# violetdenim/c3dgs

Measured on AMD Instinct MI355X. Metric: raster views/sec fwd+bwd @1920x1080, higher is better.
Workload: dtype f32; 1 GPU; BASELINE.json configs[2]: synth-v1 3M Gaussians, SH deg 3, indexed-camera rasterizer (QAT inner loop), mark_visible+fwd+bwd, 1 view/step/GPU; gaussians=3000000, width=1920, height=1080, sh_codebook=304096, gaussian_codebook=754096, parallelism=replicas x1

## Files before the change

__graft_entry__.py:

```python
import os
import subprocess
import sys

ROOT = os.path.dirname(os.path.abspath(__file__))
if ROOT not in sys.path:
    sys.path.insert(0, ROOT)


def build() -> None:
    from c3dgs_amd import build as hip_build
    lib = hip_build.build()
    assert os.path.exists(lib)
    for variant in hip_build.VARIANTS:
        assert os.path.exists(hip_build.build_variant(variant))
    subprocess.check_call(["make", "-C", os.path.join(ROOT, "oracle"), "-s"])
    import c3dgs_amd
    from c3dgs_amd import _lib
    L = _lib.lib()
    assert L.c3dgs_abi_version() == 4


def smoke() -> None:
    import numpy as np
    import torch
    from tests import cases, gpu_util, synth
    from oracle import oracle as orc

    assert torch.cuda.is_available(), "smoke() needs a GPU"
    torch.cuda.set_device(0)
    for name in ("base", "indexed"):
        inp, cam, indexed = cases.make_case(name)
        st = cases.oracle_forward(inp, cam)
        fw = gpu_util.hip_forward(inp, cam, indexed)
        u = gpu_util.unpack(fw)
        np.testing.assert_array_equal(u["radii"], st.radii)
        np.testing.assert_array_equal(u["keys_sorted"], st.keys_sorted)
        np.testing.assert_array_equal(u["point_list"], st.point_list)
        assert gpu_util.psnr(u["out_color"], st.out_color) >= 80.0
        dL = synth.grad_image(cam["W"], cam["H"]).numpy()
        ref = orc.rasterize_backward(st, dL)
        got = gpu_util.hip_backward(fw, dL)
        for k, v in got.items():
            if ref[k].shape == v.shape and v.size:
                err = gpu_util.rel_inf(v, ref[k])
                assert err <= 1e-4, (name, k, err)
    import c3dgs_amd
# ... 15 lines not shown
```

c3dgs_amd/build.py:

```python
import os
import subprocess
import sys
from concurrent.futures import ThreadPoolExecutor

HERE = os.path.dirname(os.path.abspath(__file__))
CSRC = os.path.join(HERE, "csrc")
OBJ = os.path.join(HERE, "build")
LIB = os.path.join(HERE, "libc3dgs_hip.so")
HIPCC = os.environ.get("HIPCC", "/opt/rocm/bin/hipcc")
ARCH = "gfx950"

COMMON = ["--offload-arch=" + ARCH, "-O3", "-fPIC", "-std=c++17", "-Wall", "-Wno-unused-function",
          "-fno-gpu-rdc", "-DNDEBUG"]
SOURCES = {
    "c_abi.hip": [],
    "c_abi_debug.hip": [],
    "preprocess.hip": ["-ffp-contract=off"],
    "backward_preprocess.hip": ["-ffp-contract=off"] + os.environ.get("C3DGS_BWDPRE_FLAGS", "").split(),
    "binning.hip": [],
    "radix_sort.hip": os.environ.get("C3DGS_SORT_FLAGS", "").split(),
    "render.hip": os.environ.get("C3DGS_RENDER_FLAGS", "-fno-slp-vectorize").split(),
    "vq.hip": ["-mllvm", "-amdgpu-mfma-vgpr-form"] + os.environ.get("C3DGS_VQ_FLAGS", "").split(),
    "draws.hip": [],
    "loss.hip": [],
    "metrics.hip": [],
    "encode.hip": [],
    "knn.hip": ["-ffp-contract=off"],
    "adam.hip": ["-ffp-contract=off"],
    "qat.hip": ["-ffp-contract=off"],
    "densify.hip": ["-ffp-contract=off"],
}
HEADERS = [os.path.join(CSRC, "common.hpp"), os.path.join(CSRC, "gsmath.hpp"), os.path.join(CSRC, "render_diag.hpp"),
           os.path.join(HERE, "..", "include", "c3dgs_hip.h"), os.path.join(HERE, "..", "include", "c3dgs_hip_debug.h")]


def _stale(target, deps):
    if not os.path.exists(target):
        return True
    t = os.path.getmtime(target)
    return any(os.path.getmtime(d) > t for d in deps)


def _compile(name, extra, verbose):
    src = os.path.join(CSRC, name)
    obj = os.path.join(OBJ, name.replace(".hip", ".o"))
    cmd = [HIPCC] + COMMON + extra + ["-c", src, "-o", obj]
    if verbose:
        print(" ".join(cmd), flush=True)
    subprocess.check_call(cmd)
    return obj


VARIANTS = {"spin1": {"radix_sort.hip": ["-DC3DGS_OS_SPIN_LIMIT=1u"]}}
def _diag(mode):
    return {src: ["-DC3DGS_DIAG", mode] for src in ("render.hip", "radix_sort.hip", "diag.hip")}


DIAG_VARIANTS = {"lanes": _diag("-DC3DGS_COUNT_LANES"), "bwdtime": _diag("-DC3DGS_BWD_TIMING"), "ostime": _diag("-DC3DGS_OS_TIMING")}


def build_variant(name, verbose=False):
    build(verbose=verbose)
    flags = {**VARIANTS, **DIAG_VARIANTS}[name]
    odir = os.path.join(HERE, "build", "variant_" + name)
    os.makedirs(odir, exist_ok=True)
    lib = os.path.join(HERE, f"libc3dgs_hip_{name}.so")
    objs, rebuilt = [], False
    for src in list(SOURCES) + [f for f in flags if f not in SOURCES]:
        extra = SOURCES.get(src, [])
        obj = os.path.join(OBJ, src.replace(".hip", ".o"))
        if src in flags:
            obj = os.path.join(odir, src.replace(".hip", ".o"))
            if _stale(obj, [os.path.join(CSRC, src)] + HEADERS + [os.path.abspath(__file__)]):
                cmd = [HIPCC] + COMMON + extra + flags[src] + ["-c", os.path.join(CSRC, src), "-o", obj]
                if verbose:
                    print(" ".join(cmd), flush=True)
                subprocess.check_call(cmd)
                rebuilt = True
        objs.append(obj)
    if rebuilt or _stale(lib, objs):
        subprocess.check_call([HIPCC, "--offload-arch=" + ARCH, "-shared", "-fPIC", "-o", lib] + objs)
    return lib


def build(force=False, verbose=False):
    os.makedirs(OBJ, exist_ok=True)
    deps_common = HEADERS + [os.path.abspath(__file__)]
    todo, objs = [], []
    for name, extra in SOURCES.items():
        obj = os.path.join(OBJ, name.replace(".hip", ".o"))
        objs.append(obj)
        if force or _stale(obj, [os.path.join(CSRC, name)] + deps_common):
            todo.append((name, extra))
    if todo:
        with ThreadPoolExecutor(max_workers=min(4, len(todo))) as ex:
            list(ex.map(lambda t: _compile(t[0], t[1], verbose), todo))
    if force or todo or _stale(LIB, objs):
        cmd = [HIPCC, "--offload-arch=" + ARCH, "-shared", "-fPIC", "-o", LIB] + objs
        if verbose:
            print(" ".join(cmd), flush=True)
        subprocess.check_call(cmd)
    return LIB


if __name__ == "__main__":
    print(build(force="--force" in sys.argv, verbose="--verbose" in sys.argv or "-v" in sys.argv))
    for flag, table in (("--variants", VARIANTS), ("--diag", DIAG_VARIANTS)):
        for v in table if flag in sys.argv else ():
            print(build_variant(v, verbose="--verbose" in sys.argv or "-v" in sys.argv))
```

c3dgs_amd/csrc/c_abi.hip:

```cpp
#include "common.hpp"
#include <cstdlib>
#include <cstring>
#include <mutex>
#include <vector>

namespace c3dgs {

static thread_local std::string g_last_error;
void set_error(const std::string& msg) { g_last_error = msg; }

enum Stage { ST_MARK_VISIBLE, ST_PREPROCESS, ST_DEPTH_SORT, ST_SCAN, ST_DUPLICATE, ST_SORT, ST_RANGES, ST_RENDER_FWD, ST_ZERO_PARTIALS,
             ST_RENDER_BWD, ST_BWD_PREPROCESS, ST_WDIST, ST_VQ_ACC, ST_VQ_APPLY, ST_LOSS_FWD, ST_LOSS_BWD,
             ST_QAT_OBSERVE, ST_QAT_CODEBOOKS, ST_QAT_VISIBLE, ST_QAT_POINTS, ST_QAT_POINTS_BWD, ST_QAT_CODEBOOKS_BWD, ST_ADAM,
             ST_KNN_SORT, ST_KNN_BOUNDS, ST_KNN_QUERY, ST_COUNT };
static const char* kStageNames[ST_COUNT] = { "mark_visible", "preprocess", "depth_sort", "scan", "duplicate_with_keys", "sort",
                                             "identify_ranges", "render_forward", "zero_partials", "render_backward",
                                             "backward_preprocess", "weighted_distance", "vq_accumulate", "vq_apply", "l1_ssim_forward",
                                             "l1_ssim_backward", "qat_observe", "qat_codebooks", "qat_visible", "qat_points",
                                             "qat_points_backward", "qat_codebooks_backward", "adam_step",
                                             "knn_sort", "knn_bounds", "knn_query" };
struct ProfRec { int stage; hipEvent_t a, b; };
static std::mutex g_prof_mu;
static bool g_prof_on = false;
static int g_prof_only = -1;
// ... 210 lines not shown
        const size_t n_sh = (grads->dL_dsh && p.sh) ? (size_t)p.SHS * p.M * 3 * sizeof(float) : 0;
        const size_t n_rot = (grads->dL_drotations && p.scales) ? (size_t)p.GS * 4 * sizeof(float) : 0;
        const size_t n_sc = (grads->dL_dscales && p.scales) ? (size_t)p.GS * 3 * sizeof(float) : 0;
        char* a_sh = (char*)grads->dL_dsh; char* a_rot = (char*)grads->dL_drotations; char* a_sc = (char*)grads->dL_dscales;
        if (n_sh && n_rot && n_sc && a_rot == a_sh + n_sh && a_sc == a_rot + n_rot) {
            const size_t n = n_sh + n_rot + n_sc;
            if (p.P > 0 && R >= 0 && ((uintptr_t)a_sh & 15u) == 0) {
                cb_zero = a_sh; cb_zero16 = n / 16;
                if (n % 16) C3DGS_HIP_TRY(hipMemsetAsync(a_sh + cb_zero16 * 16, 0, n % 16, s));
            } else {
                C3DGS_HIP_TRY(hipMemsetAsync(a_sh, 0, n, s));
            }
        } else {
            if (n_sh) C3DGS_HIP_TRY(hipMemsetAsync(a_sh, 0, n_sh, s));
            if (n_sc) C3DGS_HIP_TRY(hipMemsetAsync(a_sc, 0, n_sc, s));
            if (n_rot) C3DGS_HIP_TRY(hipMemsetAsync(a_rot, 0, n_rot, s));
        }
    }
    if (P == 0) return C3DGS_OK;
    if (!radii || !geom_buffer || !image_buffer || !dL_dout_color || (R > 0 && !binning_buffer))
        return fail(C3DGS_E_INVALID, "radii, forward buffers and dL_dout_color are required");
    if (!ws_resize) return fail(C3DGS_E_INVALID, "workspace callback is required");
    if (R < 0) return fail(C3DGS_E_INVALID, "R must be >= 0");

    const GeomPtrs g = geom_ptrs(const_cast<void*>(geom_buffer), P);
    const ImgPtrs img = img_ptrs(const_cast<void*>(image_buffer), W, H);
    const size_t ws_bytes = c3dgs_backward_workspace_bytes(P, R);
    float* partials = (float*)ws_resize(ws_user, ws_bytes);
    if (!partials) return fail(C3DGS_E_ALLOC, "backward workspace allocation failed");

    const size_t r1 = (size_t)(R > 0 ? R : 1), p256 = ((size_t)P + 1023) / 1024 * 1024;
    uint8_t* touched = (uint8_t*)partials + align_up(r1 * PARTIAL_FLOATS * sizeof(float));
    uint32_t* tile_order = img.tile_order;
    uint32_t* live_ids = (uint32_t*)(touched + align_up(r1)) + 65536;
    uint32_t* live_slots = live_ids + p256;
    uint32_t* live_count = live_slots + p256;
    { StageTimer t_(ST_ZERO_PARTIALS, s);
      launch_backward_prep(R > 0 ? W : 0, H, img, tile_order, touched, align_up(r1) / 16, R > 0 ? nullptr : cb_zero,
                           R > 0 ? 0 : cb_zero16, s); }
    if (R > 0) {
        const BinPtrs b = bin_ptrs(const_cast<void*>(binning_buffer), R, W, H);
        { StageTimer t_(ST_RENDER_BWD, s);
          launch_render_backward(W, H, img, g.splat, g.block_base, p.background, dL_dout_color, partials, touched,
                                 compact_ptrs(b, R, W, H), tile_order, cb_zero, cb_zero16, s); }
        C3DGS_STAGE("render_backward", p.debug, s);
    }
    { StageTimer t_(ST_BWD_PREPROCESS, s);
      launch_backward_preprocess(p, radii, g, partials, touched, live_count, live_ids, live_slots, *grads, s); }
    C3DGS_STAGE("backward_preprocess", p.debug, s);
    return C3DGS_OK;
}

}

using namespace c3dgs;

extern "C" {

const char* c3dgs_last_error(void) { return g_last_error.c_str(); }

int c3dgs_profile_enable(int on)
{
    std::lock_guard<std::mutex> lk(g_prof_mu);
    g_prof_on = on != 0;
    return C3DGS_OK;
}

int c3dgs_profile_only(const char* stage_name)
{
    std::lock_guard<std::mutex> lk(g_prof_mu);
    g_prof_only = -1;
    if (!stage_name || !*stage_name) return C3DGS_OK;
    for (int i = 0; i < ST_COUNT; i++)
        if (std::strcmp(stage_name, kStageNames[i]) == 0) { g_prof_only = i; return C3DGS_OK; }
    return fail(C3DGS_E_INVALID, std::string("profile_only: unknown stage ") + stage_name);
}

// ... 571 lines not shown
```

c3dgs_amd/csrc/common.hpp:

```cpp
#pragma once
#include <hip/hip_runtime.h>
#include <cstdint>
#include <cstddef>
#include <cstdio>
#include <cstring>
#include <string>

#include "../../include/c3dgs_hip.h"

namespace c3dgs {

constexpr int TILE = 16;
constexpr int TILE_PIX = 256;
constexpr int SPLAT_F4 = 3;
constexpr int PARTIAL_FLOATS = 9;

void set_error(const std::string& msg);
inline int fail(int code, const std::string& msg) { set_error(msg); return code; }

#define C3DGS_HIP_TRY(expr)                                                                         \
    do {                                                                                            \
        hipError_t e__ = (expr);                                                                    \
        if (e__ != hipSuccess)                                                                      \
            return ::c3dgs::fail(C3DGS_E_HIP, std::string(#expr) + ": " + hipGetErrorString(e__));  \
// ... 156 lines not shown
void launch_camera_from_pose(const float* pose, float inv_tan_x, float inv_tan_y, float* view, float* proj, float* campos, hipStream_t s);
void launch_mark_visible(int P, const float* means3D, const float* view, uint8_t* present, hipStream_t s);
void launch_mark_visible_pose(int P, const float* means3D, const float* pose7, uint8_t* present, hipStream_t s);
void launch_pack_codebook(const c3dgs_raster_params& p, float4* gtab, hipStream_t s);
void launch_preprocess(const c3dgs_raster_params& p, const GeomPtrs& g, int32_t* radii, uint2* ranges, const uint32_t* sort_err,
                       void* zero_span, size_t zero_n16, uint32_t* host_out, uint32_t host_seq, hipStream_t s);
void launch_depth_order_scan(int P, const GeomPtrs& g, hipStream_t s);
void launch_duplicate_with_keys(int P, const GeomPtrs& g, const BinPtrs& b, int grid_x, const uint32_t* sort_err,
                                void* zero_span, size_t zero_n16, hipStream_t s);
void launch_identify_ranges(int R, const void* keys_sorted, int key_bytes, uint2* ranges, const uint32_t* sort_err, hipStream_t s);
hipError_t run_depth_sort(void* temp, size_t temp_bytes, const uint32_t* kin, uint32_t* kout, const uint32_t* vin,
                          uint32_t* vout, int P, const uint2* rects, uint2* rects_sorted, hipStream_t s, bool ctrl_cleared = false,
                          bool rects_fit_bytes = false);
hipError_t run_tile_sort(void* temp, size_t temp_bytes, const void* kin, void* kout, int key_bytes, const uint32_t* vin,
                         uint32_t* vout, int R, int end_bit, hipStream_t s, bool ctrl_cleared = false);
size_t depth_sort_clear_bytes(int P);
size_t tile_sort_clear_bytes(int R, int end_bit, int key_bytes);
bool onesweep_enabled();
int onesweep_timed_out(hipStream_t s);
uint32_t* onesweep_error_word();
size_t onesweep_depth_temp_bytes(int P);
size_t onesweep_tile_temp_bytes(int R, int end_bit, int key_bytes = 2);
size_t onesweep_depth_clear_bytes(int P);
size_t onesweep_tile_clear_bytes(int R, int end_bit, int key_bytes);
hipError_t onesweep_depth_sort(void* temp, size_t temp_bytes, const uint32_t* kin, uint32_t* kout, const uint32_t* vin, uint32_t* vout,
                               int P, const uint2* gather_src, uint2* gather_dst, hipStream_t s, bool ctrl_cleared = false,
                               bool rects_fit_bytes = false);
hipError_t onesweep_tile_sort32(void* temp, size_t temp_bytes, const uint32_t* kin, uint32_t* kout, const uint32_t* vin, uint32_t* vout,
                                int R, int end_bit, hipStream_t s, bool ctrl_cleared = false);
hipError_t onesweep_tile_sort(void* temp, size_t temp_bytes, const uint16_t* kin, uint16_t* kout, const uint32_t* vin, uint32_t* vout,
                              int R, int end_bit, hipStream_t s, bool ctrl_cleared = false);
void launch_render_forward(int W, int H, const ImgPtrs& img, const uint32_t* point_list, const float4* splat,
                           const float* bg, float* out_color, const CompactPtrs& cl, const uint32_t* sort_err, hipStream_t s);
void launch_backward_prep(int W, int H, const ImgPtrs& img, uint32_t* tile_order, void* zero_a, size_t n16_a, void* zero_b,
                          size_t n16_b, hipStream_t s);
void launch_render_backward(int W, int H, const ImgPtrs& img, const float4* splat,
                            const uint32_t* block_base, const float* bg, const float* dL_dpix, float* partials,
                            uint8_t* touched, const CompactPtrs& cl, const uint32_t* tile_order, void* zero_span, size_t zero_n16,
                            hipStream_t s);
void launch_backward_preprocess(const c3dgs_raster_params& p, const int32_t* radii, const GeomPtrs& g,
                                float* partials, const uint8_t* touched, uint32_t* live_count, uint32_t* live_ids,
                                uint32_t* live_slots, const c3dgs_raster_grads& gr, hipStream_t s);
int launch_weighted_distance(int64_t N, int C, int K, const float* coefs, const int64_t* gather, const float* codebook,
                             float* out_dist, int64_t* out_idx, hipStream_t s, void* ws = nullptr, size_t ws_bytes = 0, int presplit = -1);
bool wd_presplit_supported(int C, int K, const float* coefs, const float* codebook, const void* ws, size_t ws_bytes);
int launch_vq_apply_split(int K, int D, float* S, float* codebook, float* entry_importance, float decay, float alpha, float eps,
                          int scale_normalize, void* ws, size_t ws_bytes, int parity, hipStream_t s);
void launch_vq_seed_words(int K, int D, void* ws, hipStream_t s);
uint32_t* vq_next_absmax_word(int K, int D, void* ws, int parity);
size_t wd_ws_bytes(int64_t N, int C, int K);
int launch_wd_debug_scores(int64_t N, int C, int K, const float* coefs, const float* codebook, float* scores, void* ws, size_t ws_bytes,
                           float* out_dist, int64_t* out_idx, hipStream_t s);
void launch_vq_accumulate(int64_t B, int K, int D, const float* x, const float* w, const int64_t* gather,
                          const int64_t* idx, const float* dist, float* S, double* dist_sum, hipStream_t s, uint32_t* clear_word = nullptr);
void launch_vq_apply(int K, int D, const float* S, float* codebook, float* entry_importance, float decay, float alpha,
                     float eps, int scale_normalize, hipStream_t s);

size_t morton_workspace_bytes(int P);
int run_morton_order(int P, const float* xyz, int64_t* codes_out, int64_t* order_out, void* workspace, hipStream_t s);
void launch_extract_rot_scale(int n, const float* cov6, float* rot, float* scale, hipStream_t s);
size_t knn_workspace_bytes(int P);
int run_knn_sort(int P, const float* xyz, void* workspace, hipStream_t s);
void launch_knn_bounds(int P, void* workspace, hipStream_t s);
void launch_knn_query(int P, const void* workspace, float* out, hipStream_t s);
void launch_adam(int n_tensors, const c3dgs_adam_tensor* tensors, double beta1, double beta2, double eps, hipStream_t s);
void launch_abs_accumulate(int64_t n, const float* g, float* acc, hipStream_t s);
void launch_densify_classify(int P, const float* accum, const float* denom, const float* scale_clone, const float* scale_split,
                             const float* scale_prune_self, const float* scale_prune_child, const float* opacity, float max_grad,
                             float dense_extent, float min_opacity, float big_extent, uint8_t* code, hipStream_t s);
size_t rows_plan_workspace_bytes(int P);
hipError_t run_rows_plan(int P, const uint8_t* code, int N, long long capacity, int32_t* src, uint8_t* kind, int32_t* draw_row,
// ... 41 lines not shown
```

c3dgs_amd/csrc/render.hip:

```cpp
#include "common.hpp"
#include "render_diag.hpp"
#include <algorithm>

namespace c3dgs {

constexpr int BATCH = 256;

__device__ __forceinline__ void prescale_conic(float4& a, float4& b)
{
    constexpr float LOG2E = 1.4426950408889634f;
    a.z *= -0.5f * LOG2E;
    a.w *= -LOG2E;
    b.x *= -0.5f * LOG2E;
}

__device__ __forceinline__ bool gaussian_alpha(float mx, float my, float ka, float kb, float kc, float op,
                                               float pxf, float pyf, float& dx, float& dy, float& G, float& alpha)
{
    dx = mx - pxf;
    dy = my - pyf;
    const float power2 = fmaf(kb, dx * dy, fmaf(kc, dy * dy, ka * (dx * dx)));
    G = __builtin_amdgcn_exp2f(power2);
    alpha = fminf(0.99f, op * G);
    return !(power2 > 0.0f) && !(alpha < 1.0f / 255.0f);
// ... 10 lines not shown
}

__device__ __forceinline__ uint32_t quadrant_mask(const float4 a, const float4 b, float tile_x0, float tile_y0)
{
    const float mx = a.x, my = a.y, ca = a.z, cb = a.w, cc = b.x, op = b.y;
    if (op < (1.0f / 255.0f) * 0.999f) return 0u;
    const float det = ca * cc - cb * cb;
    const float tau = __logf(255.0f * op) * 1.0001f + 1e-4f;
    if (!(det > 0.0f) || !(ca > 0.0f) || !(cc > 0.0f) || !(tau < 1e30f)) return 0xfu;
    const float nb_c = -cb / cc, nb_a = -cb / ca;
    uint32_t mask = 0u;
#pragma unroll
    for (int q = 0; q < 4; q++) {
        const float x0 = tile_x0 + (float)((q & 1) * 8) - 0.01f - mx, y0 = tile_y0 + (float)((q >> 1) * 8) - 0.01f - my;
        const float fmin = min_power_on_rect(ca, cb, cc, nb_c, nb_a, x0, x0 + 7.02f, y0, y0 + 7.02f);
        mask |= (uint32_t)(!(fmin > tau)) << q;
    }
    return mask;
}

__device__ __forceinline__ unsigned long long uniform_u64(unsigned long long v)
{
    const uint32_t lo = __builtin_amdgcn_readfirstlane((uint32_t)v), hi = __builtin_amdgcn_readfirstlane((uint32_t)(v >> 32));
    return ((unsigned long long)hi << 32) | lo;
}

__device__ __forceinline__ int tile_of_block(int b, int T)
{
    const int chunk = (T + 7) >> 3;
    return (b & 7) * chunk + (b >> 3);
}

__global__ void __launch_bounds__(1024) backward_prep_kernel(int T, const uint32_t* __restrict__ tile_used, uint32_t* __restrict__ order,
                                                              uint4* __restrict__ zero_a, size_t n16_a, uint4* __restrict__ zero_b, size_t n16_b)
{
    if (blockIdx.x > 0) {
        const uint4 z = make_uint4(0u, 0u, 0u, 0u);
        const size_t stride = (size_t)(gridDim.x - 1) * 1024;
        for (size_t i = (size_t)(blockIdx.x - 1) * 1024 + threadIdx.x; i < n16_a; i += stride) zero_a[i] = z;
        for (size_t i = (size_t)(blockIdx.x - 1) * 1024 + threadIdx.x; i < n16_b; i += stride) zero_b[i] = z;
        return;
    }
    if (T <= 0) return;
    auto work = [&](int i) { return tile_used[i]; };
    __shared__ uint32_t s_cnt[1024], s_w[16];
    const int t = threadIdx.x, lane = t & 63, wave = t >> 6;
    s_cnt[t] = 0;
    __syncthreads();
    for (int i = t; i < T; i += 1024) atomicAdd(&s_cnt[1023 - min(work(i) >> 3, 1023u)], 1u);
    __syncthreads();
    const uint32_t c = s_cnt[t];
    uint32_t incl = c;
#pragma unroll
    for (int o = 1; o < 64; o <<= 1) { const uint32_t v = __shfl_up(incl, o); if (lane >= o) incl += v; }
    if (lane == 63) s_w[wave] = incl;
    __syncthreads();
    uint32_t off = 0;
    for (int w = 0; w < wave; w++) off += s_w[w];
    s_cnt[t] = off + incl - c;
    __syncthreads();
    for (int i = t; i < T; i += 1024) order[atomicAdd(&s_cnt[1023 - min(work(i) >> 3, 1023u)], 1u)] = (uint32_t)i;
}

__global__ void __launch_bounds__(256)
render_forward_kernel(int W, int H, int gx, int T, const uint2* __restrict__ ranges, const uint32_t* __restrict__ point_list,
                      const float4* __restrict__ splat, const float* __restrict__ bg, float* __restrict__ out_color,
                      float* __restrict__ final_T, uint32_t* __restrict__ n_contrib, uint32_t* __restrict__ tile_used,
                      uint32_t* __restrict__ n_contrib_c, uint32_t* __restrict__ tile_used_c, uint8_t* __restrict__ cqm,
                      uint32_t* __restrict__ cid, const uint32_t* __restrict__ sort_err)
{
    const int tile = tile_of_block(blockIdx.x, T);
    if (tile >= T || (blockIdx.x >> 3) >= ((T + 7) >> 3)) return;
    __shared__ float4 s_ab[2][BATCH + 1][2];
    __shared__ float s_c[2][BATCH + 1];
    __shared__ uint32_t s_list[4][BATCH + 8];
    __shared__ int s_wdone[2][4];
// ... 181 lines not shown
__device__ __forceinline__ void reduce_columns_24(float* u, int lane)
{
    transpose_reduce_step<24, 0xB1>(u, (lane & 1) != 0);
    transpose_reduce_step<12, 0x4E>(u, (lane & 2) != 0);
}

__device__ __forceinline__ void reduce_rows_9(const float* n, float& total, float& ninth)
{
    float o[4];
    C3DGS_TR4("row_ror:8", "0x3", "0xc", o, n, n, 0, 4);
    float t8;
    asm volatile("s_nop 1\n\tv_add_f32_dpp %0, %1, %1 row_ror:8 row_mask:0xf bank_mask:0xf" : "=&v"(t8) : "v"(n[8]));
    auto s0 = __builtin_amdgcn_permlane16_swap(__float_as_uint(o[0]), __float_as_uint(o[2]), false, false);
    auto s1 = __builtin_amdgcn_permlane16_swap(__float_as_uint(o[1]), __float_as_uint(o[3]), false, false);
    auto s8 = __builtin_amdgcn_permlane16_swap(__float_as_uint(t8), __float_as_uint(t8), false, false);
    const float w0 = __uint_as_float(s0[0]) + __uint_as_float(s0[1]);
    const float w1 = __uint_as_float(s1[0]) + __uint_as_float(s1[1]);
    const float w8 = __uint_as_float(s8[0]) + __uint_as_float(s8[1]);
    auto s2 = __builtin_amdgcn_permlane32_swap(__float_as_uint(w0), __float_as_uint(w1), false, false);
    auto s9 = __builtin_amdgcn_permlane32_swap(__float_as_uint(w8), __float_as_uint(w8), false, false);
    total = __uint_as_float(s2[0]) + __uint_as_float(s2[1]);
    ninth = __uint_as_float(s9[0]) + __uint_as_float(s9[1]);
}

#ifndef C3DGS_BWD_WPE
#define C3DGS_BWD_WPE 5
#endif
__global__ void __launch_bounds__(256) __attribute__((amdgpu_waves_per_eu(C3DGS_BWD_WPE, C3DGS_BWD_WPE)))
render_backward_kernel(int W, int H, int gx, int T, const uint2* __restrict__ ranges, const uint32_t* __restrict__ tile_used_c,
                       const uint32_t* __restrict__ cid, const float4* __restrict__ splat,
                       const uint32_t* __restrict__ block_base, const float* __restrict__ bg, const float* __restrict__ final_Ts,
                       const uint32_t* __restrict__ n_contrib_c, const float* __restrict__ dL_dpixels,
                       float* __restrict__ partials, uint8_t* __restrict__ touched, const uint8_t* __restrict__ cqm,
                       const uint32_t* __restrict__ tile_order, uint4* __restrict__ zero_span, size_t zero_n16)
{
    if (zero_n16) {
        const size_t per = (zero_n16 + gridDim.x - 1) / gridDim.x, z0 = (size_t)blockIdx.x * per, z1 = min(z0 + per, zero_n16);
        for (size_t i = z0 + threadIdx.x; i < z1; i += 256) zero_span[i] = make_uint4(0u, 0u, 0u, 0u);
    }
    if ((int)blockIdx.x >= T) return;
    PhaseClock clk;
    const int tile = (int)tile_order[blockIdx.x];
    __shared__ float4 s_ab[BATCH + 1][2];
    __shared__ float s_c[BATCH + 1];
    __shared__ uint32_t s_slot[BATCH];
    __shared__ uint32_t s_list[4][BATCH / 2 + GROUP_G];
    __shared__ unsigned long long s_mask[4][4];
    __shared__ float s_part[2][BATCH][NPART];
    constexpr uint32_t REC_BYTES = 32;
    const char* rec_base = reinterpret_cast<const char*>(&s_ab[0][0]);
    const char* blue_base = reinterpret_cast<const char*>(&s_c[0]);

    const int tid = threadIdx.x, wave = tid >> 6, lane = tid & 63;
    const int tx = tile % gx, ty = tile / gx;
    const int px = tx * TILE + (wave & 1) * 8 + (lane & 7);
    const int py = ty * TILE + (wave >> 1) * 8 + (lane >> 3);
    const bool inside = px < W && py < H;
    const float pxf = (float)px, pyf = (float)py;
    const size_t pix = (size_t)W * py + px, HW = (size_t)H * W;

    const uint2 range = ranges[tile];
    const int n = (int)(range.y - range.x);
    const int used = min(n, (int)tile_used_c[tile]);
    if (used <= 0) return;
    const int rounds = (used + BATCH - 1) / BATCH;
    if (tid == 0) { s_ab[BATCH][0] = make_float4(0, 0, 0, 0); s_ab[BATCH][1] = make_float4(0, 0, 0, 0); s_c[BATCH] = 0.f; }
    for (int q = tid; q < 4 * (BATCH / 2 + GROUP_G); q += 256) (&s_list[0][0])[q] = (uint32_t)BATCH * REC_BYTES;

    const float T_final = inside ? final_Ts[pix] : 0.f;
    float Tr = T_final;
    const int last_contributor = inside ? (int)n_contrib_c[pix] : 0;
    float dpx0 = 0.f, dpx1 = 0.f, dpx2 = 0.f;
    if (inside) { dpx0 = dL_dpixels[pix]; dpx1 = dL_dpixels[HW + pix]; dpx2 = dL_dpixels[2 * HW + pix]; }
    float Sd = T_final * (bg[0] * dpx0 + bg[1] * dpx1 + bg[2] * dpx2);
    int wave_last = last_contributor;
#pragma unroll
    for (int o = 32; o > 0; o >>= 1) wave_last = max(wave_last, __shfl_xor(wave_last, o));
    wave_last = __builtin_amdgcn_readfirstlane(wave_last);
    const int beta = ((lane >> 2) & 1) * 4 + (lane & 1) * 2 + ((lane >> 1) & 1);
    const int my_m = ((lane >> 3) & 1) * 4 + ((lane >> 4) & 1) * 2 + ((lane >> 5) & 1);
    LaneCount lc;

    uint32_t next_id = 0u, next_qm = 0u;
    {
        const int p0 = used - 1 - tid;
        if (p0 >= 0) { next_id = cid[range.x + p0]; next_qm = cqm[range.x + p0]; }
    }
    clk.mark(PhaseClock::PROLOGUE);
    for (int r = 0; r < rounds; r++) {
        __syncthreads();
        clk.mark(PhaseClock::TOP_BARRIER);
        const int mypos = used - 1 - (r * BATCH + tid);
        uint32_t qm = 0u;
        if (mypos >= 0) {
            const uint32_t id = next_id;
            qm = next_qm;
            float4 a = splat[3 * (size_t)id], b = splat[3 * (size_t)id + 1];
            const float4 c = splat[3 * (size_t)id + 2];
            prescale_conic(a, b);
            const uint32_t off = __float_as_uint(c.y), lo = __float_as_uint(c.z), hi = __float_as_uint(c.w);
            const int x0 = lo & 0xffff, y0 = lo >> 16, x1 = hi & 0xffff;
            s_slot[tid] = block_base[id >> 8] + off + (uint32_t)((ty - y0) * (x1 - x0) + (tx - x0));
            s_ab[tid][0] = a; s_ab[tid][1] = b; s_c[tid] = c.x;
        }
        {
            const int npos = mypos - BATCH;
            if (npos >= 0) { next_id = cid[range.x + npos]; next_qm = cqm[range.x + npos]; }
        }
#pragma unroll
        for (int q = 0; q < 4; q++) {
            const unsigned long long bm = __ballot((qm >> q) & 1u);
            if (lane == 0) s_mask[q][wave] = bm;
        }
        clk.mark(PhaseClock::GATHER);
#pragma unroll
        for (int w = 0; w < 2; w++)
#pragma unroll
            for (int q = 0; q < NPART; q++) s_part[w][tid][q] = 0.f;
        clk.mark(PhaseClock::CLEAR);
        __syncthreads();
        clk.mark(PhaseClock::CLOSE_BARRIER);

        const int cnt = min(BATCH, used - r * BATCH);
        const int pos0 = used - 1 - r * BATCH;
        const int thr = (pos0 - last_contributor) * (int)REC_BYTES;
#pragma unroll 1
        for (int half = 0; half < 2; half++) {
        int nw = 0;
        {
            const unsigned long long lt = (1ull << lane) - 1ull;
#pragma unroll
            for (int cc = 0; cc < 2; cc++) {
                const int c = half * 2 + cc;
                unsigned long long m = uniform_u64(s_mask[wave][c]);
                const int jmin = pos0 - wave_last + 1 - c * 64;
                if (jmin >= 64) m = 0; else if (jmin > 0) m &= ~0ull << jmin;
                if ((m >> lane) & 1ull) s_list[wave][nw + (int)__popcll(m & lt)] = (uint32_t)(c * 64 + lane) * REC_BYTES;
                nw += (int)__popcll(m);
            }
            if (lane < GROUP_G) s_list[wave][nw + lane] = (uint32_t)BATCH * REC_BYTES;
            __builtin_amdgcn_fence(__ATOMIC_RELEASE, "wavefront");
            __builtin_amdgcn_wave_barrier();
            __builtin_amdgcn_fence(__ATOMIC_ACQUIRE, "wavefront");
        }
        clk.mark(PhaseClock::COMPACT);
        uint4 row0 = *reinterpret_cast<const uint4*>(&s_list[wave][0]);
        uint4 row1 = *reinterpret_cast<const uint4*>(&s_list[wave][4]);
        float4 a_n = *reinterpret_cast<const float4*>(rec_base + row0.x);
        float4 b_n = *reinterpret_cast<const float4*>(rec_base + row0.x + 16);
        float c_n = *reinterpret_cast<const float*>(blue_base + (row0.x >> 3));
        for (int k = 0; k < nw; k += GROUP_G) {
            const uint32_t* lrow = &s_list[wave][k];
            const uint32_t e[GROUP_G] = { row0.x, row0.y, row0.z, row0.w, row1.x, row1.y, row1.z, row1.w };
            float v[GROUP_G * NCOL];
// ... 23 lines not shown
                v[g * NCOL + 2] = dchannel_dcolor * dpx2;
                const float dL_dalpha = fmaf(Tr, cd, -(rinv * Sd));
                Sd = fmaf(dchannel_dcolor, cd, Sd);
                const float w = G_eff * dL_dalpha, wx = w * dx;
                v[g * NCOL + 3] = w;
                v[g * NCOL + 4] = wx;
                v[g * NCOL + 5] = wx * dx;
                if (g == 4) { C3DGS_TR4("row_half_mirror", "0x5", "0xa", u, v, v, 0, 24); }
                if (g == 5) { C3DGS_TR4("row_half_mirror", "0x5", "0xa", u, v, v, 4, 24); C3DGS_TR4("row_half_mirror", "0x5", "0xa", u, v, v, 8, 24); }
                if (g == 6) { C3DGS_TR4("row_half_mirror", "0x5", "0xa", u, v, v, 12, 24); }
                if (g == 7) { C3DGS_TR4("row_half_mirror", "0x5", "0xa", u, v, v, 16, 24); C3DGS_TR4("row_half_mirror", "0x5", "0xa", u, v, v, 20, 24); }
            }
            row0 = *reinterpret_cast<const uint4*>(lrow + GROUP_G);
            row1 = *reinterpret_cast<const uint4*>(lrow + GROUP_G + 4);
            reduce_columns_24(u, lane);
            a_n = *reinterpret_cast<const float4*>(rec_base + row0.x);
            b_n = *reinterpret_cast<const float4*>(rec_base + row0.x + 16);
            c_n = *reinterpret_cast<const float*>(blue_base + (row0.x >> 3));
            const int myj = (int)(my_off >> 5);
            const float dyb = *reinterpret_cast<const float*>(rec_base + my_off + 4) - pyf;
            float total, ninth;
            const float nine[NPART] = { u[0], u[1], u[2], u[3], u[4], u[5], dyb * u[3], dyb * u[4], (dyb * dyb) * u[3] };
            reduce_rows_9(nine, total, ninth);
            if (myj < BATCH) {
                __hip_atomic_fetch_add(&s_part[wave >> 1][myj][my_m], total, __ATOMIC_RELAXED, __HIP_MEMORY_SCOPE_WORKGROUP);
                if (lane < 8) __hip_atomic_fetch_add(&s_part[wave >> 1][myj][8], ninth, __ATOMIC_RELAXED, __HIP_MEMORY_SCOPE_WORKGROUP);
            }
        }
        lc.end_list();
        __builtin_amdgcn_fence(__ATOMIC_RELEASE, "wavefront");
        __builtin_amdgcn_wave_barrier();
        clk.mark(PhaseClock::GROUPS);
        }
        __syncthreads();
        clk.mark(PhaseClock::FLUSH_BARRIER);
        if (tid < cnt) {
            const uint32_t slot = s_slot[tid];
            float* dst = partials + (size_t)slot * NPART;
            float t[NPART];
#pragma unroll
            for (int q = 0; q < NPART; q++) t[q] = s_part[0][tid][q] + s_part[1][tid][q];
            dst[0] = t[0]; dst[1] = t[1]; dst[2] = t[2];
            dst[3] = t[3]; dst[4] = t[4]; dst[5] = t[6];
            dst[6] = t[5]; dst[7] = t[7]; dst[8] = t[8];
            touched[slot] = 1;
        }
        clk.mark(PhaseClock::FLUSH_STORES);
    }
    lc.flush(8, lane);
    clk.flush(lane);
}

void launch_backward_prep(int W, int H, const ImgPtrs& img, uint32_t* tile_order, void* zero_a, size_t n16_a, void* zero_b,
                          size_t n16_b, hipStream_t s)
{
    const int T = (W > 0 && H > 0 && tile_order) ? tiles_x(W) * tiles_y(H) : 0;
    const size_t n16 = n16_a + n16_b;
    if (T <= 0 && n16 == 0) return;
    const unsigned fill = n16 ? (unsigned)std::min<size_t>((n16 + 1023) / 1024, 1024) : 0u;
    backward_prep_kernel<<<1 + fill, 1024, 0, s>>>(T, img.tile_used_c, tile_order, (uint4*)zero_a, n16_a, (uint4*)zero_b, n16_b);
}

void launch_render_backward(int W, int H, const ImgPtrs& img, const float4* splat,
                            const uint32_t* block_base, const float* bg, const float* dL_dpix, float* partials,
                            uint8_t* touched, const CompactPtrs& cl, const uint32_t* tile_order, void* zero_span, size_t zero_n16,
                            hipStream_t s)
{
    const int gx = tiles_x(W), T = gx * tiles_y(H);
    const int grid = ((T + 7) / 8) * 8;
    render_backward_kernel<<<grid, 256, 0, s>>>(W, H, gx, T, img.ranges, img.tile_used_c, cl.cid, splat, block_base, bg, img.final_T,
                                                img.n_contrib_c, dL_dpix, partials, touched, cl.cqm, tile_order, (uint4*)zero_span,
                                                zero_span ? zero_n16 : 0);
}

}
```

c3dgs_amd/csrc/render_diag.hpp:

```cpp
#pragma once

namespace c3dgs {

#if (defined(C3DGS_COUNT_LANES) || defined(C3DGS_BWD_TIMING)) && !defined(C3DGS_DIAG)
#error "C3DGS_COUNT_LANES / C3DGS_BWD_TIMING are modes of a -DC3DGS_DIAG build"
#endif

#ifdef C3DGS_DIAG
__device__ unsigned long long g_lane_counters[16];

int read_lane_counters(unsigned long long* out16, hipStream_t s)
{
    static const unsigned long long zeros[16] = { 0 };
    if (hipStreamSynchronize(s) != hipSuccess) return 1;
    if (hipMemcpyFromSymbol(out16, HIP_SYMBOL(g_lane_counters), sizeof(zeros)) != hipSuccess) return 1;
    return hipMemcpyToSymbol(HIP_SYMBOL(g_lane_counters), zeros, sizeof(zeros)) != hipSuccess;
}
#endif

#ifdef C3DGS_COUNT_LANES
struct LaneCount {
    unsigned long long pairs = 0, slots = 0, lanes = 0, live = 0, half = 0, blk = 0, lists = 0, aux = 0;
    int nA = 0, nB = 0, nb[4] = { 0, 0, 0, 0 };
    __device__ void pair(bool real, unsigned long long used, unsigned long long aux_mask)
// ... 4 lines not shown
        lanes += __popcll(used);
        aux += __popcll(aux_mask);
        live += used != 0;
        nA += (used & 0x00000000ffffffffull) != 0;
        nB += (used & 0xffffffff00000000ull) != 0;
        nb[0] += (used & 0x000000000f0f0f0full) != 0;
        nb[1] += (used & 0x00000000f0f0f0f0ull) != 0;
        nb[2] += (used & 0x0f0f0f0f00000000ull) != 0;
        nb[3] += (used & 0xf0f0f0f000000000ull) != 0;
    }
    __device__ void end_list()
    {
        lists++;
        half += max(nA, nB);
        blk += max(max(nb[0], nb[1]), max(nb[2], nb[3]));
        nA = nB = nb[0] = nb[1] = nb[2] = nb[3] = 0;
    }
    __device__ void flush(int base, int lane)
    {
        if (lane != 0) return;
        const unsigned long long v[8] = { pairs, slots, lanes, live, half, blk, lists, aux };
        for (int q = 0; q < 8; q++) atomicAdd(&g_lane_counters[base + q], v[q]);
    }
};
#else
struct LaneCount {
    __device__ __forceinline__ void pair(bool, unsigned long long, unsigned long long) {}
    __device__ __forceinline__ void end_list() {}
    __device__ __forceinline__ void flush(int, int) {}
};
#endif

struct PhaseClock {
    enum Phase { PROLOGUE, TOP_BARRIER, GATHER, CLEAR, CLOSE_BARRIER, COMPACT, GROUPS, FLUSH_BARRIER, FLUSH_STORES, NPHASE };
#ifdef C3DGS_BWD_TIMING
    unsigned long long born = __builtin_readcyclecounter(), last = born, sum[NPHASE] = {};
    __device__ void mark(Phase p)
    {
        const unsigned long long now = __builtin_readcyclecounter();
        sum[p] += now - last;
        last = now;
    }
    __device__ void flush(int lane)
    {
        if (lane != 0) return;
        for (int p = 0; p < NPHASE; p++) atomicAdd(&g_lane_counters[p], sum[p]);
        atomicAdd(&g_lane_counters[9], (unsigned long long)__builtin_readcyclecounter() - born);
        atomicAdd(&g_lane_counters[10], 1ull);
    }
#else
    __device__ __forceinline__ void mark(Phase) {}
    __device__ __forceinline__ void flush(int) {}
#endif
};

}
```

Measured before the change: 618.9 views/s.

## Make backward render kernel persistent with atomic tile ticket and next-tile prefetch

The backward rasterizer now launches at most as many workgroups as can be resident, and each workgroup loops over tiles it takes from a global atomic ticket, initialised in the prep kernel, walking the precomputed tile order. While finishing the current tile it prefetches the next tile's range, first-batch ids and per-pixel inputs, to hide the launch and prologue latency between tiles and balance uneven tile costs. This adds an atomic per tile, extra registers and shared state, and a dependence on occupancy queries. Grid-cap build variants are also added for experiments.

```diff
diff --git a/__graft_entry__.py b/__graft_entry__.py
--- a/__graft_entry__.py
+++ b/__graft_entry__.py
@@ -11,7 +11,7 @@
     from c3dgs_amd import build as hip_build
     lib = hip_build.build()
     assert os.path.exists(lib)
-    for variant in hip_build.VARIANTS:
+    for variant in list(hip_build.VARIANTS) + list(hip_build.GRID_VARIANTS):
         assert os.path.exists(hip_build.build_variant(variant))
     subprocess.check_call(["make", "-C", os.path.join(ROOT, "oracle"), "-s"])
     import c3dgs_amd
diff --git a/c3dgs_amd/build.py b/c3dgs_amd/build.py
--- a/c3dgs_amd/build.py
+++ b/c3dgs_amd/build.py
@@ -52,6 +52,7 @@
 
 
 VARIANTS = {"spin1": {"radix_sort.hip": ["-DC3DGS_OS_SPIN_LIMIT=1u"]}}
+GRID_VARIANTS = {"bwdgrid1": {"render.hip": ["-DC3DGS_BWD_GRID=1"]}, "bwdgrid3": {"render.hip": ["-DC3DGS_BWD_GRID=3"]}}
 def _diag(mode):
     return {src: ["-DC3DGS_DIAG", mode] for src in ("render.hip", "radix_sort.hip", "diag.hip")}
 
@@ -61,7 +62,7 @@
 
 def build_variant(name, verbose=False):
     build(verbose=verbose)
-    flags = {**VARIANTS, **DIAG_VARIANTS}[name]
+    flags = {**VARIANTS, **GRID_VARIANTS, **DIAG_VARIANTS}[name]
     odir = os.path.join(HERE, "build", "variant_" + name)
     os.makedirs(odir, exist_ok=True)
     lib = os.path.join(HERE, f"libc3dgs_hip_{name}.so")
@@ -105,6 +106,6 @@
 
 if __name__ == "__main__":
     print(build(force="--force" in sys.argv, verbose="--verbose" in sys.argv or "-v" in sys.argv))
-    for flag, table in (("--variants", VARIANTS), ("--diag", DIAG_VARIANTS)):
+    for flag, table in (("--variants", {**VARIANTS, **GRID_VARIANTS}), ("--diag", DIAG_VARIANTS)):
         for v in table if flag in sys.argv else ():
             print(build_variant(v, verbose="--verbose" in sys.argv or "-v" in sys.argv))
diff --git a/c3dgs_amd/csrc/c_abi.hip b/c3dgs_amd/csrc/c_abi.hip
--- a/c3dgs_amd/csrc/c_abi.hip
+++ b/c3dgs_amd/csrc/c_abi.hip
@@ -266,17 +266,18 @@
     const size_t r1 = (size_t)(R > 0 ? R : 1), p256 = ((size_t)P + 1023) / 1024 * 1024;
     uint8_t* touched = (uint8_t*)partials + align_up(r1 * PARTIAL_FLOATS * sizeof(float));
     uint32_t* tile_order = img.tile_order;
-    uint32_t* live_ids = (uint32_t*)(touched + align_up(r1)) + 65536;
+    uint32_t* bwd_ticket = (uint32_t*)(touched + align_up(r1));
+    uint32_t* live_ids = bwd_ticket + 65536;
     uint32_t* live_slots = live_ids + p256;
     uint32_t* live_count = live_slots + p256;
     { StageTimer t_(ST_ZERO_PARTIALS, s);
-      launch_backward_prep(R > 0 ? W : 0, H, img, tile_order, touched, align_up(r1) / 16, R > 0 ? nullptr : cb_zero,
+      launch_backward_prep(R > 0 ? W : 0, H, img, tile_order, bwd_ticket, touched, align_up(r1) / 16, R > 0 ? nullptr : cb_zero,
                            R > 0 ? 0 : cb_zero16, s); }
     if (R > 0) {
         const BinPtrs b = bin_ptrs(const_cast<void*>(binning_buffer), R, W, H);
         { StageTimer t_(ST_RENDER_BWD, s);
           launch_render_backward(W, H, img, g.splat, g.block_base, p.background, dL_dout_color, partials, touched,
-                                 compact_ptrs(b, R, W, H), tile_order, cb_zero, cb_zero16, s); }
+                                 compact_ptrs(b, R, W, H), tile_order, bwd_ticket, cb_zero, cb_zero16, s); }
         C3DGS_STAGE("render_backward", p.debug, s);
     }
     { StageTimer t_(ST_BWD_PREPROCESS, s);
diff --git a/c3dgs_amd/csrc/common.hpp b/c3dgs_amd/csrc/common.hpp
--- a/c3dgs_amd/csrc/common.hpp
+++ b/c3dgs_amd/csrc/common.hpp
@@ -212,11 +212,11 @@
                               int R, int end_bit, hipStream_t s, bool ctrl_cleared = false);
 void launch_render_forward(int W, int H, const ImgPtrs& img, const uint32_t* point_list, const float4* splat,
                            const float* bg, float* out_color, const CompactPtrs& cl, const uint32_t* sort_err, hipStream_t s);
-void launch_backward_prep(int W, int H, const ImgPtrs& img, uint32_t* tile_order, void* zero_a, size_t n16_a, void* zero_b,
+void launch_backward_prep(int W, int H, const ImgPtrs& img, uint32_t* tile_order, uint32_t* ticket, void* zero_a, size_t n16_a, void* zero_b,
                           size_t n16_b, hipStream_t s);
 void launch_render_backward(int W, int H, const ImgPtrs& img, const float4* splat,
                             const uint32_t* block_base, const float* bg, const float* dL_dpix, float* partials,
-                            uint8_t* touched, const CompactPtrs& cl, const uint32_t* tile_order, void* zero_span, size_t zero_n16,
+                            uint8_t* touched, const CompactPtrs& cl, const uint32_t* tile_order, uint32_t* ticket, void* zero_span, size_t zero_n16,
                             hipStream_t s);
 void launch_backward_preprocess(const c3dgs_raster_params& p, const int32_t* radii, const GeomPtrs& g,
                                 float* partials, const uint8_t* touched, uint32_t* live_count, uint32_t* live_ids,
diff --git a/c3dgs_amd/csrc/render.hip b/c3dgs_amd/csrc/render.hip
--- a/c3dgs_amd/csrc/render.hip
+++ b/c3dgs_amd/csrc/render.hip
@@ -66,7 +66,8 @@
 }
 
 __global__ void __launch_bounds__(1024) backward_prep_kernel(int T, const uint32_t* __restrict__ tile_used, uint32_t* __restrict__ order,
-                                                              uint4* __restrict__ zero_a, size_t n16_a, uint4* __restrict__ zero_b, size_t n16_b)
+                                                              uint4* __restrict__ zero_a, size_t n16_a, uint4* __restrict__ zero_b, size_t n16_b,
+                                                              uint32_t* __restrict__ ticket)
 {
     if (blockIdx.x > 0) {
         const uint4 z = make_uint4(0u, 0u, 0u, 0u);
@@ -76,6 +77,7 @@
         return;
     }
     if (T <= 0) return;
+    if (threadIdx.x == 0) *ticket = 0u;
     auto work = [&](int i) { return tile_used[i]; };
     __shared__ uint32_t s_cnt[1024], s_w[16];
     const int t = threadIdx.x, lane = t & 63, wave = t >> 6;
@@ -323,60 +325,89 @@
                        const uint32_t* __restrict__ block_base, const float* __restrict__ bg, const float* __restrict__ final_Ts,
                        const uint32_t* __restrict__ n_contrib_c, const float* __restrict__ dL_dpixels,
                        float* __restrict__ partials, uint8_t* __restrict__ touched, const uint8_t* __restrict__ cqm,
-                       const uint32_t* __restrict__ tile_order, uint4* __restrict__ zero_span, size_t zero_n16)
+                       const uint32_t* __restrict__ tile_order, uint4* __restrict__ zero_span, size_t zero_n16,
+                       uint32_t* __restrict__ ticket)
 {
     if (zero_n16) {
         const size_t per = (zero_n16 + gridDim.x - 1) / gridDim.x, z0 = (size_t)blockIdx.x * per, z1 = min(z0 + per, zero_n16);
         for (size_t i = z0 + threadIdx.x; i < z1; i += 256) zero_span[i] = make_uint4(0u, 0u, 0u, 0u);
     }
+    const int G = (int)gridDim.x;
     if ((int)blockIdx.x >= T) return;
     PhaseClock clk;
-    const int tile = (int)tile_order[blockIdx.x];
     __shared__ float4 s_ab[BATCH + 1][2];
     __shared__ float s_c[BATCH + 1];
     __shared__ uint32_t s_slot[BATCH];
     __shared__ uint32_t s_list[4][BATCH / 2 + GROUP_G];
     __shared__ unsigned long long s_mask[4][4];
     __shared__ float s_part[2][BATCH][NPART];
+    __shared__ uint32_t s_next[2];
     constexpr uint32_t REC_BYTES = 32;
     const char* rec_base = reinterpret_cast<const char*>(&s_ab[0][0]);
     const char* blue_base = reinterpret_cast<const char*>(&s_c[0]);
 
     const int tid = threadIdx.x, wave = tid >> 6, lane = tid & 63;
-    const int tx = tile % gx, ty = tile / gx;
-    const int px = tx * TILE + (wave & 1) * 8 + (lane & 7);
-    const int py = ty * TILE + (wave >> 1) * 8 + (lane >> 3);
-    const bool inside = px < W && py < H;
-    const float pxf = (float)px, pyf = (float)py;
-    const size_t pix = (size_t)W * py + px, HW = (size_t)H * W;
-
-    const uint2 range = ranges[tile];
-    const int n = (int)(range.y - range.x);
-    const int used = min(n, (int)tile_used_c[tile]);
-    if (used <= 0) return;
-    const int rounds = (used + BATCH - 1) / BATCH;
     if (tid == 0) { s_ab[BATCH][0] = make_float4(0, 0, 0, 0); s_ab[BATCH][1] = make_float4(0, 0, 0, 0); s_c[BATCH] = 0.f; }
     for (int q = tid; q < 4 * (BATCH / 2 + GROUP_G); q += 256) (&s_list[0][0])[q] = (uint32_t)BATCH * REC_BYTES;
-
-    const float T_final = inside ? final_Ts[pix] : 0.f;
-    float Tr = T_final;
-    const int last_contributor = inside ? (int)n_contrib_c[pix] : 0;
-    float dpx0 = 0.f, dpx1 = 0.f, dpx2 = 0.f;
-    if (inside) { dpx0 = dL_dpixels[pix]; dpx1 = dL_dpixels[HW + pix]; dpx2 = dL_dpixels[2 * HW + pix]; }
-    float Sd = T_final * (bg[0] * dpx0 + bg[1] * dpx1 + bg[2] * dpx2);
-    int wave_last = last_contributor;
-#pragma unroll
-    for (int o = 32; o > 0; o >>= 1) wave_last = max(wave_last, __shfl_xor(wave_last, o));
-    wave_last = __builtin_amdgcn_readfirstlane(wave_last);
     const int beta = ((lane >> 2) & 1) * 4 + (lane & 1) * 2 + ((lane >> 1) & 1);
     const int my_m = ((lane >> 3) & 1) * 4 + ((lane >> 4) & 1) * 2 + ((lane >> 5) & 1);
     LaneCount lc;
 
+    int px = 0, py = 0, last_contributor = 0;
+    float Tr = 0.f, dpx0 = 0.f, dpx1 = 0.f, dpx2 = 0.f;
     uint32_t next_id = 0u, next_qm = 0u;
-    {
-        const int p0 = used - 1 - tid;
-        if (p0 >= 0) { next_id = cid[range.x + p0]; next_qm = cqm[range.x + p0]; }
-    }
+    const size_t HW = (size_t)H * W;
+    auto tile_scalars = [&](int tl, uint32_t& first, int& len) {
+        const uint2 range = ranges[tl];
+        first = range.x;
+        len = min((int)(range.y - range.x), (int)tile_used_c[tl]);
+    };
+    auto load_first_batch = [&](uint32_t first, int len) {
+        asm volatile("" : "+s"(len));
+        const int p0 = len - 1 - tid;
+        if (p0 >= 0) { next_id = cid[first + p0]; next_qm = cqm[first + p0]; }
+    };
+    auto load_pixels = [&](int tl) {
+        asm volatile("" : "+s"(tl));
+        px = (tl % gx) * TILE + (wave & 1) * 8 + (lane & 7);
+        py = (tl / gx) * TILE + (wave >> 1) * 8 + (lane >> 3);
+        const bool in = px < W && py < H;
+        const size_t pix = (size_t)W * py + px;
+        Tr = in ? final_Ts[pix] : 0.f;
+        last_contributor = in ? (int)n_contrib_c[pix] : 0;
+        dpx0 = 0.f; dpx1 = 0.f; dpx2 = 0.f;
+        if (in) { dpx0 = dL_dpixels[pix]; dpx1 = dL_dpixels[HW + pix]; dpx2 = dL_dpixels[2 * HW + pix]; }
+    };
+
+    int tile = (int)tile_order[blockIdx.x];
+    int k_nxt = 2 * G - 1 - (int)blockIdx.x;
+    uint32_t first = 0u, par = 0u;
+    int used = 0;
+    tile_scalars(tile, first, used);
+    if (used > 0) { load_first_batch(first, used); load_pixels(tile); }
+
+    for (;;) {
+    const bool more = k_nxt < T;
+    uint32_t drawn = 0u;
+    if (more && tid == 0) drawn = atomicAdd(ticket, 1u);
+    const int tile_n = more ? (int)tile_order[k_nxt] : 0;
+    uint32_t first_n = 0u;
+    int used_n = 0;
+    auto next_scalars_and_publish = [&]() {
+        if (more) tile_scalars(tile_n, first_n, used_n);
+        if (more && tid == 0) s_next[par] = (uint32_t)(2 * G) + drawn;
+    };
+    if (used > 0) {
+    clk.tile();
+    const int tx = tile % gx, ty = tile / gx;
+    const float pxf = (float)px, pyf = (float)py;
+    const float T_final = Tr;
+    float Sd = T_final * (bg[0] * dpx0 + bg[1] * dpx1 + bg[2] * dpx2);
+    int wave_last = last_contributor;
+#pragma unroll
+    for (int o = 32; o > 0; o >>= 1) wave_last = max(wave_last, __shfl_xor(wave_last, o));
+    wave_last = __builtin_amdgcn_readfirstlane(wave_last);
+    const int rounds = (used + BATCH - 1) / BATCH;
     clk.mark(PhaseClock::PROLOGUE);
     for (int r = 0; r < rounds; r++) {
         __syncthreads();
@@ -396,7 +427,7 @@
         }
         {
             const int npos = mypos - BATCH;
-            if (npos >= 0) { next_id = cid[range.x + npos]; next_qm = cqm[range.x + npos]; }
+            if (npos >= 0) { next_id = cid[first + npos]; next_qm = cqm[first + npos]; }
         }
 #pragma unroll
         for (int q = 0; q < 4; q++) {
@@ -404,6 +435,8 @@
             if (lane == 0) s_mask[q][wave] = bm;
         }
         clk.mark(PhaseClock::GATHER);
+        if (r == 0) next_scalars_and_publish();
+        clk.mark(PhaseClock::NEXT_TILE);
 #pragma unroll
         for (int w = 0; w < 2; w++)
 #pragma unroll
@@ -411,6 +444,8 @@
         clk.mark(PhaseClock::CLEAR);
         __syncthreads();
         clk.mark(PhaseClock::CLOSE_BARRIER);
+        if (r == rounds - 1 && used_n > 0) load_first_batch(first_n, used_n);
+        clk.mark(PhaseClock::NEXT_TILE);
 
         const int cnt = min(BATCH, used - r * BATCH);
         const int pos0 = used - 1 - r * BATCH;
@@ -500,6 +535,8 @@
         __builtin_amdgcn_wave_barrier();
         clk.mark(PhaseClock::GROUPS);
         }
+        if (r == rounds - 1 && used_n > 0) load_pixels(tile_n);
+        clk.mark(PhaseClock::NEXT_TILE);
         __syncthreads();
         clk.mark(PhaseClock::FLUSH_BARRIER);
         if (tid < cnt) {
@@ -515,30 +552,59 @@
         }
         clk.mark(PhaseClock::FLUSH_STORES);
     }
+    } else {
+        next_scalars_and_publish();
+        __syncthreads();
+        if (used_n > 0) { load_first_batch(first_n, used_n); load_pixels(tile_n); }
+    }
+    if (!more) break;
+    k_nxt = (int)__builtin_amdgcn_readfirstlane(s_next[par]);
+    par ^= 1u;
+    tile = tile_n; first = first_n; used = used_n;
+    }
     lc.flush(8, lane);
     clk.flush(lane);
 }
 
-void launch_backward_prep(int W, int H, const ImgPtrs& img, uint32_t* tile_order, void* zero_a, size_t n16_a, void* zero_b,
-                          size_t n16_b, hipStream_t s)
+void launch_backward_prep(int W, int H, const ImgPtrs& img, uint32_t* tile_order, uint32_t* ticket, void* zero_a, size_t n16_a,
+                          void* zero_b, size_t n16_b, hipStream_t s)
 {
     const int T = (W > 0 && H > 0 && tile_order) ? tiles_x(W) * tiles_y(H) : 0;
     const size_t n16 = n16_a + n16_b;
     if (T <= 0 && n16 == 0) return;
     const unsigned fill = n16 ? (unsigned)std::min<size_t>((n16 + 1023) / 1024, 1024) : 0u;
-    backward_prep_kernel<<<1 + fill, 1024, 0, s>>>(T, img.tile_used_c, tile_order, (uint4*)zero_a, n16_a, (uint4*)zero_b, n16_b);
+    backward_prep_kernel<<<1 + fill, 1024, 0, s>>>(T, img.tile_used_c, tile_order, (uint4*)zero_a, n16_a, (uint4*)zero_b, n16_b, ticket);
+}
+
+static int backward_resident_workgroups()
+{
+    static int cache[64] = { 0 };
+    int dev = 0;
+    if (hipGetDevice(&dev) != hipSuccess || dev < 0 || dev >= 64) return 0;
+    if (!cache[dev]) {
+        int occ = 0, cus = 0;
+        if (hipOccupancyMaxActiveBlocksPerMultiprocessor(&occ, render_backward_kernel, 256, 0) != hipSuccess) return 0;
+        if (hipDeviceGetAttribute(&cus, hipDeviceAttributeMultiprocessorCount, dev) != hipSuccess) return 0;
+        cache[dev] = std::max(occ, 0) * std::max(cus, 0);
+    }
+    return cache[dev];
 }
 
 void launch_render_backward(int W, int H, const ImgPtrs& img, const float4* splat,
                             const uint32_t* block_base, const float* bg, const float* dL_dpix, float* partials,
-                            uint8_t* touched, const CompactPtrs& cl, const uint32_t* tile_order, void* zero_span, size_t zero_n16,
-                            hipStream_t s)
+                            uint8_t* touched, const CompactPtrs& cl, const uint32_t* tile_order, uint32_t* ticket, void* zero_span,
+                            size_t zero_n16, hipStream_t s)
 {
     const int gx = tiles_x(W), T = gx * tiles_y(H);
-    const int grid = ((T + 7) / 8) * 8;
+    if (T <= 0) return;
+    const int resident = backward_resident_workgroups();
+    int grid = resident > 0 ? std::min(T, resident) : T;
+#ifdef C3DGS_BWD_GRID
+    grid = std::min(grid, C3DGS_BWD_GRID);
+#endif
     render_backward_kernel<<<grid, 256, 0, s>>>(W, H, gx, T, img.ranges, img.tile_used_c, cl.cid, splat, block_base, bg, img.final_T,
                                                 img.n_contrib_c, dL_dpix, partials, touched, cl.cqm, tile_order, (uint4*)zero_span,
-                                                zero_span ? zero_n16 : 0);
-}
-
-}
+                                                zero_span ? zero_n16 : 0, ticket);
+}
+
+}
diff --git a/c3dgs_amd/csrc/render_diag.hpp b/c3dgs_amd/csrc/render_diag.hpp
--- a/c3dgs_amd/csrc/render_diag.hpp
+++ b/c3dgs_amd/csrc/render_diag.hpp
@@ -60,9 +60,12 @@
 #endif
 
 struct PhaseClock {
-    enum Phase { PROLOGUE, TOP_BARRIER, GATHER, CLEAR, CLOSE_BARRIER, COMPACT, GROUPS, FLUSH_BARRIER, FLUSH_STORES, NPHASE };
+    enum Phase { PROLOGUE, TOP_BARRIER, GATHER, CLEAR, CLOSE_BARRIER, COMPACT, GROUPS, FLUSH_BARRIER, FLUSH_STORES,
+                 NEXT_TILE,
+                 NPHASE };
 #ifdef C3DGS_BWD_TIMING
-    unsigned long long born = __builtin_readcyclecounter(), last = born, sum[NPHASE] = {};
+    unsigned long long born = __builtin_readcyclecounter(), last = born, sum[NPHASE] = {}, tiles = 0;
+    __device__ void tile() { tiles++; }
     __device__ void mark(Phase p)
     {
         const unsigned long long now = __builtin_readcyclecounter();
@@ -73,11 +76,13 @@
     {
         if (lane != 0) return;
         for (int p = 0; p < NPHASE; p++) atomicAdd(&g_lane_counters[p], sum[p]);
-        atomicAdd(&g_lane_counters[9], (unsigned long long)__builtin_readcyclecounter() - born);
         atomicAdd(&g_lane_counters[10], 1ull);
+        atomicAdd(&g_lane_counters[11], (unsigned long long)__builtin_readcyclecounter() - born);
+        atomicAdd(&g_lane_counters[12], tiles);
     }
 #else
     __device__ __forceinline__ void mark(Phase) {}
+    __device__ __forceinline__ void tile() {}
     __device__ __forceinline__ void flush(int) {}
 #endif
 };
```

Result: slower. 602.4 views/s (-2.7%).
